# kkromberg/SpeechRecognition

Measured on AMD Instinct MI355X. Metric: frames/sec scored+decoded, higher is better.
Workload: dtype f64

## Files before the change

### speechrecognition_amd/csrc/gmm_prefilter.hip

```cpp
#include <hip/hip_runtime.h>
#include <stdint.h>

#include <algorithm>
#include <cmath>
#include <vector>

#include "kernels.h"

#ifndef SR_P16_NB
#define SR_P16_NB 4
#endif

namespace srgpu {

typedef float v4f __attribute__((ext_vector_type(4)));
static constexpr int kPWaves = 4;
static constexpr int kGroupBlocks = 8;

typedef _Float16 f16x8 __attribute__((ext_vector_type(8)));

__device__ inline uint32_t pack_f16x2(_Float16 l, _Float16 h) {
  return (uint32_t)__builtin_bit_cast(uint16_t, l) | ((uint32_t)__builtin_bit_cast(uint16_t, h) << 16);
}

template <int KS32, int NB>
__global__ __launch_bounds__(kPWaves * 64, (NB <= 2 ? 3 : 2)) void gmm_prefilter16_kernel(GmmPrefilterArgs a) {
  constexpr int kBlockBytes = KS32 * 1024;
  constexpr int kStageBytes = kGroupBlocks * kBlockBytes;
  constexpr int kChunksPerStage = kStageBytes / 1024;
  constexpr int kDmaPerWave = kChunksPerStage / kPWaves;
  static_assert(kChunksPerStage % kPWaves == 0, "every wave issues the same number of LDS-DMA pieces per stage");
  constexpr int kTileFrames = kPWaves * NB * 16;
  constexpr size_t kTileBytes = (size_t)kTileFrames * (16 * KS32) * sizeof(float);
  constexpr size_t kLdsBytes = 2 * kStageBytes > kTileBytes ? 2 * kStageBytes : kTileBytes;
  __shared__ __attribute__((aligned(1024))) unsigned char lds[kLdsBytes];

  const int lane = threadIdx.x & 63, wave = threadIdx.x >> 6;
  const int g = lane >> 4, c = lane & 15;
  uint32_t x, y;
  {
    const uint32_t id = blockIdx.x;
    if ((a.ny & 7u) == 0) { const uint32_t j = id >> 3; y = (id & 7u) + 8u * (j / a.nx); x = j % a.nx; }
    else { y = id / a.nx; x = id % a.nx; }
  }
  const uint32_t g0 = a.split_begin[y], g1 = a.split_begin[y + 1];
  const uint64_t frame0 = (uint64_t)x * kTileFrames + (uint64_t)wave * (NB * 16);

  uint4 bf[NB][KS32];
  float bnorm[NB], dbnorm[NB];
  {
    float* fl = reinterpret_cast<float*>(lds);
    const uint64_t tile_first = (uint64_t)x * kTileFrames;
    const uint64_t tile_frames = (a.n_frames - tile_first < (uint64_t)kTileFrames) ? a.n_frames - tile_first : kTileFrames;
    const uint32_t n_floats = (uint32_t)tile_frames * a.dim;
    const float* src = a.feats + tile_first * a.dim;
    for (uint32_t i = threadIdx.x; i < n_floats; i += kPWaves * 64) fl[i] = src[i];
    __syncthreads();
#pragma unroll
    for (int nb = 0; nb < NB; nb++) {
      const uint32_t row = (uint32_t)wave * (NB * 16) + nb * 16 + c;
      const bool valid = row < tile_frames;
      const float* xr = fl + (valid ? row : 0u) * a.dim;
      float n2 = 0.0f, e2 = 0.0f;
#pragma unroll
      for (int ks = 0; ks < KS32; ks++) {
        _Float16 v[8];
#pragma unroll
        for (int j = 0; j < 8; j++) {
          const uint32_t k = 32u * ks + 8u * g + j, d = k >> 1;
          const float xf = (valid && d < a.dim) ? xr[d < a.dim ? d : 0u] : 0.0f;
          const float b = (k & 1u) ? xf : xf * xf;
          n2 += b * b;
          _Float16 h = (_Float16)b;
          const float bh = (float)h;
          const float e = (k & 1u) ? xf - bh : __builtin_fmaf(xf, xf, -bh);
          e2 += e * e;
          if (valid && k >= 2u * a.dim && k < 2u * a.dim + 3u) h = (_Float16)1.0f;
          v[j] = h;
        }
        bf[nb][ks] = make_uint4(pack_f16x2(v[0], v[1]), pack_f16x2(v[2], v[3]), pack_f16x2(v[4], v[5]), pack_f16x2(v[6], v[7]));
      }
      n2 += __shfl_xor(n2, 16);
      n2 += __shfl_xor(n2, 32);
      e2 += __shfl_xor(e2, 16);
      e2 += __shfl_xor(e2, 32);
      bnorm[nb] = sqrtf(n2) * 1.0001f;
      dbnorm[nb] = fminf(sqrtf(e2) * 1.0001f, kPfRes16 * bnorm[nb]);
    }
    __syncthreads();
  }

  const unsigned char* dma_src = a.apack + (uint64_t)g0 * kStageBytes + (uint64_t)wave * 1024 + lane * 16;
  auto issue_stage = [&](int buf) {
#pragma unroll
    for (int i = 0; i < kDmaPerWave; i++) {
      const int chunk = i * kPWaves + wave;
      unsigned char* dst = lds + buf * kStageBytes + chunk * 1024;
      __builtin_amdgcn_global_load_lds((const __attribute__((address_space(1))) void*)(dma_src + i * (kPWaves * 1024)),
                                       (__attribute__((address_space(3))) void*)dst, 16, 0, 0);
    }
    dma_src += kStageBytes;
  };
  auto frag = [&](int buf, int j, int ks) -> f16x8 {
    return __builtin_bit_cast(f16x8, *reinterpret_cast<const uint4*>(lds + buf * kStageBytes + j * kBlockBytes + ks * 1024 + lane * 16));
  };

  const uint32_t n_stages = g1 - g0;
  if (n_stages > 0) issue_stage(0);
  if (n_stages > 1) issue_stage(1);
  if (n_stages > 1) __builtin_amdgcn_s_waitcnt(0x0F70 | kDmaPerWave);
  else __builtin_amdgcn_s_waitcnt(0x0F70);
  __syncthreads();
  f16x8 a_c, a_n;
  if (n_stages > 0) a_c = frag(0, 0, 0);
  uint32_t* m_ptr = a.mask + (uint64_t)g0 * a.n_frames * 4u;
  uint32_t m_off[NB];
  bool m_ok[NB];
#pragma unroll
  for (int nb = 0; nb < NB; nb++) {
    const uint64_t f = frame0 + (uint64_t)nb * 16 + c;
    m_ok[nb] = f < a.n_frames;
    m_off[nb] = (uint32_t)f * 4u + (uint32_t)g;
  }
  for (uint32_t s = 0; s < n_stages; s++) {
    const uint32_t grp = g0 + s;
    const int buf = s & 1;
    v4f ap[NB][kGroupBlocks];
#pragma unroll
    for (int j = 0; j < kGroupBlocks; j++) {
      v4f acc[NB];
#pragma unroll
      for (int nb = 0; nb < NB; nb++) acc[nb] = (v4f){0.f, 0.f, 0.f, 0.f};
#pragma unroll
      for (int ks = 0; ks < KS32; ks++) {
        if (j == kGroupBlocks - 1 && ks == KS32 - 1) {
          if (s + 1 < n_stages) {
            __builtin_amdgcn_s_waitcnt(0x0070);
            __syncthreads();
            if (s + 2 < n_stages) issue_stage(buf);
            a_n = frag(buf ^ 1, 0, 0);
          }
        } else {
          a_n = frag(buf, (ks == KS32 - 1) ? j + 1 : j, (ks == KS32 - 1) ? 0 : ks + 1);
        }
        __builtin_amdgcn_sched_barrier(0);
#pragma unroll
        for (int nb = 0; nb < NB; nb++)
          acc[nb] = __builtin_amdgcn_mfma_f32_16x16x32_f16(a_c, __builtin_bit_cast(f16x8, bf[nb][ks]), acc[nb], 0, 0, 0);
        __builtin_amdgcn_sched_barrier(0);
        a_c = a_n;
      }
#pragma unroll
      for (int nb = 0; nb < NB; nb++) ap[nb][j] = acc[nb];
    }
    const float4 lim = reinterpret_cast<const float4*>(a.grp_lim)[4u * grp + g];
#pragma unroll
    for (int nb = 0; nb < NB; nb++) {
      float amin = __builtin_huge_valf();
#pragma unroll
      for (int j = 0; j < kGroupBlocks; j += 2)
        asm("v_min3_f32 %0, %0, %1, %2\n\tv_min3_f32 %0, %0, %3, %4\n\tv_min3_f32 %0, %0, %5, %6\n\tv_min3_f32 %0, %0, %7, %8"
            : "+v"(amin)
            : "v"(ap[nb][j][0]), "v"(ap[nb][j][1]), "v"(ap[nb][j][2]), "v"(ap[nb][j][3]), "v"(ap[nb][j + 1][0]),
              "v"(ap[nb][j + 1][1]), "v"(ap[nb][j + 1][2]), "v"(ap[nb][j + 1][3]));
      if (a.chunks >= 2) { const float o = __shfl_xor(amin, 16); asm("v_min_f32 %0, %0, %1" : "+v"(amin) : "v"(o)); }
      if (a.chunks >= 4) { const float o = __shfl_xor(amin, 32); asm("v_min_f32 %0, %0, %1" : "+v"(amin) : "v"(o)); }
      const float limit = amin + __builtin_fmaf(lim.y, dbnorm[nb], __builtin_fmaf(lim.x, bnorm[nb], lim.z));
      uint32_t mask = 0;
#pragma unroll
      for (int j = kGroupBlocks - 1; j >= 1; j -= 2)
        asm("v_cmp_ngt_f32 vcc, %2, %1\n\tv_addc_co_u32 %0, vcc, %0, %0, vcc\n\t"
            "v_cmp_ngt_f32 vcc, %3, %1\n\tv_addc_co_u32 %0, vcc, %0, %0, vcc\n\t"
            "v_cmp_ngt_f32 vcc, %4, %1\n\tv_addc_co_u32 %0, vcc, %0, %0, vcc\n\t"
            "v_cmp_ngt_f32 vcc, %5, %1\n\tv_addc_co_u32 %0, vcc, %0, %0, vcc\n\t"
            "v_cmp_ngt_f32 vcc, %6, %1\n\tv_addc_co_u32 %0, vcc, %0, %0, vcc\n\t"
            "v_cmp_ngt_f32 vcc, %7, %1\n\tv_addc_co_u32 %0, vcc, %0, %0, vcc\n\t"
            "v_cmp_ngt_f32 vcc, %8, %1\n\tv_addc_co_u32 %0, vcc, %0, %0, vcc\n\t"
            "v_cmp_ngt_f32 vcc, %9, %1\n\tv_addc_co_u32 %0, vcc, %0, %0, vcc"
            : "+v"(mask)
            : "v"(limit), "v"(ap[nb][j][3]), "v"(ap[nb][j][2]), "v"(ap[nb][j][1]), "v"(ap[nb][j][0]), "v"(ap[nb][j - 1][3]),
              "v"(ap[nb][j - 1][2]), "v"(ap[nb][j - 1][1]), "v"(ap[nb][j - 1][0])
            : "vcc");
      if (m_ok[nb]) m_ptr[m_off[nb]] = mask;
    }
    m_ptr += a.n_frames * 4u;
  }
}

__global__ void fp16_denormal_probe_kernel(float* out) {
  const int lane = threadIdx.x;
  f16x8 a = {0, 0, 0, 0, 0, 0, 0, 0}, b = {0, 0, 0, 0, 0, 0, 0, 0};
  if (lane < 16) { a[0] = (_Float16)9.5367431640625e-7f; b[0] = (_Float16)1024.0f; }
  v4f acc = {0.f, 0.f, 0.f, 0.f};
  acc = __builtin_amdgcn_mfma_f32_16x16x32_f16(a, b, acc, 0, 0, 0);
  out[lane] = acc[0];
}

hipError_t probe_fp16_denormals(hipStream_t stream, bool* preserved) {
  float* d = nullptr;
  hipError_t e = hipMalloc(reinterpret_cast<void**>(&d), 64 * sizeof(float));
  if (e != hipSuccess) return e;
  hipLaunchKernelGGL(fp16_denormal_probe_kernel, dim3(1), dim3(64), 0, stream, d);
  float h[64];
  e = hipGetLastError();
  if (e == hipSuccess) e = hipStreamSynchronize(stream);
  if (e == hipSuccess) e = hipMemcpy(h, d, sizeof(h), hipMemcpyDeviceToHost);
  (void)hipFree(d);
  if (e != hipSuccess) return e;
  *preserved = true;
  for (int i = 0; i < 64; i++) *preserved = *preserved && h[i] == 9.765625e-4f;
  return hipSuccess;
}

template <int KS>
__global__ void fp16_accumulation_probe_kernel(const _Float16* A, const _Float16* B, float* out) {
  constexpr int K = 32 * KS;
  const int lane = threadIdx.x, r = lane & 15, q = lane >> 4;
  v4f acc = {0.f, 0.f, 0.f, 0.f};
#pragma unroll
// ... 616 lines not shown
#pragma unroll 1
    for (uint32_t pos = 0; pos < n_left; pos += 64u) {
      const RingEntry en = nxt;
      const uint32_t n = n_left - pos < 64u ? n_left - pos : 64u;
      const uint32_t p2 = pos + 64u;
      if (p2 < n_left) nxt = sj[p2 + ((uint32_t)lane < n_left - p2 ? lane : 0)];
      batch(true, j, en, (uint32_t)lane < n);
      level2(false);
    }
  }
  level2(true);
  if (a.n_refined) {
    if (lane == 0) atomicAdd(a.n_refined, (unsigned long long)n_eval);
  }
}

__device__ inline uint32_t padded_source_dim(uint32_t k, uint32_t dim, uint32_t dp) {
  const uint32_t pairs = dim - (dim & 1u);
  return k < pairs ? k : (k == dp - 1u && (dim & 1u)) ? dim - 1u : dim;
}
__global__ void transpose_feats_kernel(const float* feats, uint64_t n_frames, uint32_t dim, uint32_t dp, uint64_t ldT, float* out, float* featsP) {
  __shared__ float tile[64][65];
  const uint64_t f0 = (uint64_t)blockIdx.x * 64;
  for (uint32_t d0 = 0; d0 < dp; d0 += 64) {
    for (uint32_t i = threadIdx.x; i < 64 * 64; i += blockDim.x) {
      const uint32_t fr = i / 64, d = i % 64;
      const uint32_t src = d0 + d < dp ? padded_source_dim(d0 + d, dim, dp) : dim;
      tile[fr][d] = (f0 + fr < n_frames && src < dim) ? feats[(f0 + fr) * dim + src] : 0.0f;
    }
    __syncthreads();
    for (uint32_t i = threadIdx.x; i < 64 * 64; i += blockDim.x) {
      const uint32_t d = i / 64, fr = i % 64;
      if (f0 + fr < n_frames && d0 + d < dp) out[(uint64_t)(d0 + d) * ldT + f0 + fr] = tile[fr][d];
    }
    if (featsP) {
      for (uint32_t i = threadIdx.x; i < 64 * 64; i += blockDim.x) {
        const uint32_t fr = i / 64, d = i % 64;
        if (f0 + fr < n_frames && d0 + d < dp) featsP[(f0 + fr) * dp + d0 + d] = tile[fr][d];
      }
    }
    __syncthreads();
  }
}

hipError_t launch_transpose_feats(const float* feats, uint64_t n_frames, uint32_t dim, uint32_t dp, uint64_t ldT, float* out, float* featsP,
                                  hipStream_t stream) {
  if (n_frames == 0) return hipSuccess;
  if (dp < dim || (dp != dim && !featsP)) return hipErrorInvalidValue;
  hipLaunchKernelGGL(transpose_feats_kernel, dim3((unsigned)((n_frames + 63) / 64)), dim3(256), 0, stream, feats, n_frames, dim, dp, ldT, out,
                     dp != dim ? featsP : nullptr);
  return hipGetLastError();
}

int gmm_refine_slots(uint32_t max_dens, uint32_t padded_dim) { return padded_dim > 39 ? 32 : max_dens <= 8 ? 8 : max_dens <= 16 ? 16 : 32; }

uint32_t gmm_refine_padded_dim(uint32_t dim) {
  static const uint32_t bounds[] = {9, 17, 25, 33, 39, 47, 55, 63};
  const uint32_t need = dim | 1u;
  for (uint32_t b : bounds)
    if (need <= b) return b;
  return 0;
}

static int refine_threads(uint32_t dp) { return dp <= 47 ? kRThreads : kRThreadsWide; }
static int refine_spw(const GmmRefineArgs& a) {
  return (size_t)(2 * a.dim + 2) * a.n_slots * 8 * 8 <= 160 * 1024 ? 8 : 4;
}
static void refine_grid(const GmmRefineArgs& a, int spw, uint32_t* n_sgroups, uint64_t* splits, uint64_t* frames_per_split) {
  const uint64_t nt = (uint64_t)refine_threads(a.dim);
  *n_sgroups = (a.n_pstates + spw - 1) / spw;
  uint64_t sp = std::max<uint64_t>(1, (512 + *n_sgroups - 1) / *n_sgroups);
  sp = std::min<uint64_t>(sp, (a.n_frames + nt - 1) / nt);
  sp = std::max<uint64_t>(sp, 1);
  *frames_per_split = (a.n_frames + sp - 1) / sp;
  *splits = *frames_per_split ? (a.n_frames + *frames_per_split - 1) / *frames_per_split : 1;
}
size_t gmm_refine_ring_words(const GmmRefineArgs& a) {
  uint32_t g; uint64_t sp, fps;
  refine_grid(a, refine_spw(a), &g, &sp, &fps);
  return (size_t)g * sp * kRWaves * kRingWave;
}

static uint32_t defer_cap_for(const GmmRefineArgs& a, int spw) {
  uint32_t g; uint64_t sp, fps;
  refine_grid(a, spw, &g, &sp, &fps);
  const uint64_t per_wave = ((fps + kRThreads - 1) / kRThreads) * 64;
  return (uint32_t)std::min<uint64_t>(((per_wave / 4 + 63) & ~(uint64_t)63) + 64, 1u << 30);
}
void gmm_refine_defer_layout(const GmmRefineArgs& a, size_t budget_bytes, uint32_t cap_limit, uint32_t* cap, size_t* n_entries,
                             size_t* n_counts) {
  *cap = 0; *n_entries = 0; *n_counts = 0;
  if (a.chunks < 2 || a.dim > 39 || a.n_slots != 32 || a.n_frames == 0) return;
  uint32_t g; uint64_t sp, fps;
  refine_grid(a, 8, &g, &sp, &fps);
  uint32_t c = defer_cap_for(a, 8);
  if (cap_limit) c = std::min(c, cap_limit);
  const size_t segs = (size_t)g * sp * kRWaves * 8;
  if (segs * c * 16 > budget_bytes) return;
  *cap = c; *n_entries = segs * c; *n_counts = segs;
}

template <int DT, int NS, int SPW, int CH, int NT, int VS = 1>
static hipError_t launch_refine_one(const GmmRefineArgs& a0, hipStream_t stream) {
  GmmRefineArgs a = a0;
  const size_t state_bytes = (size_t)(2 * DT + 2) * NS * 8;
  const size_t smem = (SPW * state_bytes + 1023) & ~(size_t)1023;
// ... 69 lines not shown
```

### speechrecognition_amd/csrc/handles.h

```cpp
#pragma once
#include <hip/hip_runtime.h>

#include <atomic>
#include <condition_variable>
#include <cstdint>
#include <map>
#include <memory>
#include <mutex>
#include <string>
#include <thread>
#include <vector>

#include "../../include/srgpu.h"
#include "host_util.h"
#include "kernels.h"

namespace srhost {
int fail(int code, const char* fmt, ...) __attribute__((format(printf, 2, 3)));
}

#define HIP_TRY(expr)                                                                             \
  do {                                                                                            \
    hipError_t e_ = (expr);                                                                       \
    if (e_ != hipSuccess) return srhost::fail(SR_EHIP, "%s: %s (%s:%d)", #expr, hipGetErrorString(e_), __FILE__, __LINE__); \
// ... 13 lines not shown
  }
  hipError_t upload(const T* src, size_t count) {
    hipError_t e = ensure(count);
    if (e != hipSuccess || count == 0) return e;
    return hipMemcpy(p, src, count * sizeof(T), hipMemcpyHostToDevice);
  }
  void release() { if (p) (void)hipFree(p); p = nullptr; n = 0; }
  void swap(DevBuf& o) { T* tp = p; p = o.p; o.p = tp; size_t tn = n; n = o.n; o.n = tn; }
  DevBuf() = default;
  DevBuf(const DevBuf&) = delete;
  DevBuf& operator=(const DevBuf&) = delete;
  ~DevBuf() { release(); }
};

struct EventPair { hipEvent_t a, b; int kind; };


struct sr_feeder;


struct CorpusSpare {
  DevBuf<float> feats;
  DevBuf<uint64_t> d_frame_off;
  DevBuf<uint32_t> utt_order, out_words, out_count, out_flags;
  DevBuf<double> tb_score;
  DevBuf<uint16_t> tb_word, tb_bkp;
  size_t bytes() const {
    return feats.n * 4 + d_frame_off.n * 8 + (utt_order.n + out_words.n + out_count.n + out_flags.n) * 4 + tb_score.n * 8 + (tb_word.n + tb_bkp.n) * 2;
  }
};
size_t corpus_spare_cap_bytes();

struct sr_model {
  int device = 0;
  uint32_t dim = 0, n_states = 0, ld = 0;
  uint64_t n_dens = 0;
  bool max_approx = true;
  DevBuf<uint32_t> dens_off;
  DevBuf<double> means, inv_vars, norm, logw;
  DevBuf<uint32_t> dens_mean, dens_var;
  std::vector<uint32_t> h_dens_off, h_dens_mean, h_dens_var;
  std::vector<double> h_means, h_inv_vars, h_norm, h_logw;
  bool mfma_packed = false, pf_packed = false;
  uint32_t n_mean = 0, n_var = 0;
  int ksteps = 0;
  uint32_t n_blocks = 0, n_groups = 0;
  DevBuf<double> apack;
  DevBuf<uint32_t> blk_meta, grp_state;
  std::vector<uint32_t> group_first_block;
  std::map<uint32_t, std::unique_ptr<DevBuf<uint32_t>>> split_tabs, pf_split_tabs;
  const uint32_t *split_cur = nullptr, *pf_split_cur = nullptr;
  uint32_t split_ny = 0;
  int pf_ks32 = 0;
  uint32_t pf_groups = 0, pf_ny = 0, max_dens = 0, pf_slots = 0, pf_chunks = 1, pf_pstates = 0;
  DevBuf<unsigned char> pf_apack;
  DevBuf<float> pf_lim, featsT, featsP;
  DevBuf<uint4> pf_defer;
  DevBuf<uint32_t> pf_defer_cnt;
  int neg_possible = -1;
  uint32_t pf_dp = 0;
  DevBuf<uint32_t> pf_mask, pf_ndens, pf_ring;
  DevBuf<double> pf_rows;
  DevBuf<unsigned long long> pf_counter;
  hipStream_t s_copy = nullptr;
  float* staging[2] = {nullptr, nullptr};
  hipEvent_t staging_free[2] = {nullptr, nullptr};
  std::atomic<bool> staging_busy{false};
  std::mutex spare_mu;
  std::unique_ptr<CorpusSpare> spare;
  std::vector<sr_corpus*> corpora;
  hipStream_t s_gmm = nullptr, s_search = nullptr;
  DevBuf<double> scores[2];
  hipEvent_t ev_scored[2] = {nullptr, nullptr}, ev_consumed[2] = {nullptr, nullptr};
  size_t chunk_frames = 0;
  bool overlap = true;
  size_t defer_budget = (size_t)32 << 30;
  uint32_t defer_cap_limit = 0;
  size_t fb_budget = (size_t)1 << 30;
  bool profiling = false;
  std::vector<EventPair> events;
  sr_profile prof{};
};

struct sr_corpus {
  sr_model* model = nullptr;
  sr_feeder* feeder = nullptr;
  uint32_t n_utts = 0;
  uint64_t n_frames = 0;
  std::vector<uint64_t> frame_off;
  DevBuf<float> feats;
  DevBuf<uint64_t> d_frame_off;
  DevBuf<uint32_t> utt_order;
  size_t order_chunk_frames = 0;
  DevBuf<double> tb_score;
  DevBuf<uint16_t> tb_word, tb_bkp;
  DevBuf<uint32_t> out_words, out_count, out_flags;
  DevBuf<unsigned char> big_ws;
  DevBuf<uint16_t> automata, out_states;
  DevBuf<uint64_t> aut_off, bp_off, al_blk_frame0;
  DevBuf<uint32_t> al_list_off, al_states, al_blk_frames, al_blk_list;
  DevBuf<uint8_t> backptr;
  DevBuf<double> out_cost, path_scores;
  DevBuf<uint64_t> pair_off;
  DevBuf<uint32_t> pair_frame, key_mean, key_var, iota, keys_sorted, pairs_sorted, row_begin;
  DevBuf<double> pair_w, acc_mean, acc_var, w_mean, w_var;
  bool acc_valid = false;
  uint32_t acc_n_mean = 0, acc_n_var = 0;
  DevBuf<unsigned char> sort_temp;
  DevBuf<double> fb_trellis, fb_item_w, fb_weight;
// ... 144 lines not shown
```

### speechrecognition_amd/csrc/kernels.h

```cpp
#pragma once
#include <hip/hip_runtime.h>
#include <stdint.h>

#include <vector>

namespace srgpu {

struct GmmMfmaArgs {
  const float* feats;
  uint64_t n_frames;
  uint32_t dim;
  const double* apack;
  const uint32_t* blk_meta;
  const uint32_t* grp_state;
  const uint32_t* split_begin;
  double* out;
  uint32_t ld;
  uint32_t nx, ny;
};
int gmm_mfma_ksteps_for_dim(uint32_t dim);
int gmm_mfma_frames_per_tile(int ksteps);
hipError_t launch_gmm_mfma(const GmmMfmaArgs& a, int ksteps, bool sum, hipStream_t stream);

struct GmmExactArgs {
  const float* feats;
  uint64_t n_frames;
  uint32_t dim;
  uint32_t n_states;
  const uint32_t* dens_off;
  const double* means;
  const double* inv_vars;
  const double* norm;
  const double* logw;
  double* out;
  uint32_t ld;
  uint32_t states_per_split;
};
hipError_t launch_gmm_exact(const GmmExactArgs& a, bool sum, uint32_t n_splits, hipStream_t stream);
struct GmmExactList {
  const uint64_t* blk_frame0;
  const uint32_t* blk_frames;
  const uint32_t* blk_list;
  const uint32_t* list_off;
  const uint32_t* states;
  uint32_t blk_first;
  uint64_t frame_base;
};
hipError_t launch_gmm_exact_listed(const GmmExactArgs& a, bool sum, const GmmExactList& L, uint32_t n_blocks, hipStream_t stream);
int gmm_exact_frames_per_block();

struct GmmPrefilterArgs {
  const float* feats;
  uint64_t n_frames;
  uint32_t dim;
  const unsigned char* apack;
  const float* grp_lim;
  const uint32_t* split_begin;
  uint32_t* mask;
  uint32_t nx, ny;
  uint32_t chunks;
};
struct PfBound { float kappa, acc, abs, sub; };
constexpr float kPfRes16 = 4.8835e-4f;
inline constexpr PfBound pf_bound(int ks32) {
  return ks32 == 4 ? PfBound{1.05e-3f, 1.6e-5f, 7.0e-7f, 3.38e-7f} : PfBound{1.05e-3f, 1.1e-5f, 6.0e-7f, 2.92e-7f};
}
struct GmmRefineArgs {
  const float* feats;
  const float* featsT;
  uint64_t n_frames, n_frames_ld;
  uint32_t dim, n_pstates, chunks;
  const uint32_t* n_dens_ps;
  const double* rows;
  uint32_t n_slots;
  const uint32_t* mask;
  double* out; uint32_t ld;
  uint64_t frames_per_split;
  unsigned long long* n_refined;
  uint32_t* ring;
  void* defer;
  uint32_t* defer_cnt;
  uint32_t defer_cap;
};
void gmm_refine_defer_layout(const GmmRefineArgs& a, size_t budget_bytes, uint32_t cap_limit, uint32_t* cap, size_t* n_entries,
                             size_t* n_counts);
size_t gmm_refine_ring_words(const GmmRefineArgs& a);
hipError_t launch_gmm_prefilter(const GmmPrefilterArgs& a, int ks32, hipStream_t stream);
int gmm_prefilter_frames_per_tile();
hipError_t probe_fp16_denormals(hipStream_t stream, bool* preserved);
hipError_t probe_fp16_accumulation(hipStream_t stream, int ks32, bool* ok, double* worst_ratio);
uint32_t gmm_refine_padded_dim(uint32_t dim);
int gmm_refine_slots(uint32_t max_dens, uint32_t padded_dim);
hipError_t launch_gmm_refine(const GmmRefineArgs& a, hipStream_t stream);
hipError_t launch_transpose_feats(const float* feats, uint64_t n_frames, uint32_t dim, uint32_t dp, uint64_t ldT, float* out, float* featsP,
                                  hipStream_t stream);

struct DecodeNet {
  uint32_t n_slots;
  uint32_t n_words;
  const uint32_t* slot_info;
  const uint32_t* slot_word;
  const uint32_t* word_end_slot;
  uint32_t silence_word;
  double tdp_loop, tdp_forward, tdp_skip;
  uint32_t silence_state;
};
static constexpr uint32_t kSlotPos0 = 1u << 16;
static constexpr uint32_t kSlotPos1 = 1u << 17;
static constexpr uint32_t kSlotEnd = 1u << 18;
static constexpr uint32_t kSlotSilState = 1u << 19;
static constexpr uint32_t kSlotSilWord = 1u << 20;
static constexpr uint32_t kSlotFirstSil = 1u << 21;
static constexpr uint32_t kSlotSingle = 1u << 22;
struct FastNet {
  uint32_t n_slots;
  const uint32_t* state;
  const uint32_t* pred;
  const uint32_t* orig;
  const uint32_t* chunk_type;
  const uint32_t* word;
  uint32_t init_slot;
  uint32_t init_is_end;
};
struct WordNet {
  const uint32_t* info;
  const uint2* states;
  const uint32_t* order;
  uint32_t nw, nt;
  uint32_t plain_len;
  uint32_t has_general;
  uint32_t init_is_end;
};
struct DecodeArgs {
  DecodeNet net;
  FastNet fast;
  WordNet words;
  const double* scores;
  uint32_t ld;
  const uint64_t* frame_off;
  uint64_t frame_base;
// ... 525 lines not shown
```

### speechrecognition_amd/csrc/srgpu_api.cpp

```cpp
#include <hip/hip_runtime.h>

#include <algorithm>
#include <cmath>
#include <cstdarg>
#include <cstdio>
#include <cstdlib>
#include <cstring>
#include <limits>
#include <map>
#include <memory>
#include <mutex>
#include <numeric>
#include <queue>
#include <set>
#include <string>
#include <vector>

#include "../../include/srgpu.h"
#include "fb_plan.h"
#include "host_util.h"
#include "kernels.h"
#include "traceback.h"

using namespace srgpu;
// ... 212 lines not shown
          const double c = (real || t == 0) ? half_value(half_bits(rest)) : 0.0;
          arow[2 * D + t] = c;
          rest -= c;
        }
        for (int ks = 0; ks < KS; ks++)
          for (uint32_t kk = 0; kk < 32; kk++) {
            const uint32_t k = 32 * ks + kk;
            const double v = arow[k];
            const uint32_t lane = r + 16 * (kk >> 3), e = kk & 7;
            ap[(b * blk_bytes) / 2 + (size_t)ks * 512 + (size_t)lane * 8 + e] = half_bits(v);
          }
      }
    }
  }
  });
  if (Cs > 1) {
    for (uint32_t st = 0; st < S; st++)
      for (int f = 0; f < kNF; f++) {
        float mxv = 0.0f;
        for (uint32_t ch = 0; ch < Cs; ch++) {
          const float v = anorm[kNF * (size_t)(st * Cs + ch) + f];
          if (!(v <= mxv)) mxv = v;
        }
        for (uint32_t ch = 0; ch < Cs; ch++) anorm[kNF * (size_t)(st * Cs + ch) + f] = mxv;
      }
  }
  HIP_TRY(m->pf_apack.upload(reinterpret_cast<const unsigned char*>(ap.data()), ap.size() * 2));
  {
    const PfBound B = pf_bound(KS);
    for (size_t slot = 0; slot < 4 * (size_t)n_groups; slot++) {
      float* v = &anorm[kNF * slot];
      const float na = v[0], nk = v[1], nd = v[2], nh = v[3];
      const float lim0 = 2.0f * (B.acc * nk + B.abs * na), lim1_norm = 2.0f * (B.kappa * na + B.abs);
      const float lim1_res = up(2.0 * ((double)nd + (double)B.acc * nh + (double)B.abs)), limd_res = up(2.0 * (1.0 + (double)B.acc) * nh);
      const bool res = (double)limd_res * kPfRes16 + lim1_res <= lim1_norm * (1.0 - 0x1p-12) &&
                       (1.0 + (double)B.acc) * (double)B.sub * nh <= (double)B.abs * na;
      v[0] = res ? lim1_res : lim1_norm;
      v[1] = res ? limd_res : 0.0f;
      v[2] = lim0;
      v[3] = 0.0f;
    }
  }
  HIP_TRY(m->pf_lim.upload(anorm.data(), anorm.size()));
  m->pf_groups = n_groups;
  m->pf_ks32 = KS;
  m->pf_ny = 0;
  return SR_OK;
}

int set_prefilter_splits(sr_model* m, uint32_t nx) {
  const uint32_t target_wgs = 16 * 768;
  uint32_t ny = (target_wgs + nx - 1) / std::max(1u, nx);
  ny = std::max(1u, std::min(ny, std::max(1u, m->pf_groups / 8)));
  if (ny >= 8) ny &= ~7u;
  auto it = m->pf_split_tabs.find(ny);
  if (it == m->pf_split_tabs.end() || !it->second || !it->second->p) {
    std::vector<uint32_t> sb(ny + 1);
    for (uint32_t y = 0; y <= ny; y++) sb[y] = (uint32_t)((uint64_t)m->pf_groups * y / ny);
    std::unique_ptr<DevBuf<uint32_t>> fresh(new DevBuf<uint32_t>());
    HIP_TRY(fresh->upload(sb.data(), sb.size()));
    it = m->pf_split_tabs.insert_or_assign(ny, std::move(fresh)).first;
  }
  m->pf_split_cur = it->second->p;
  m->pf_ny = ny;
  return SR_OK;
}

int set_splits(sr_model* m, uint32_t nx) {
  const uint32_t target_wgs = 32 * 512;
  uint32_t ny = (target_wgs + nx - 1) / std::max(1u, nx);
  ny = std::max(1u, std::min(ny, std::min(m->n_groups, std::max(1u, m->n_blocks / 32))));
  if (ny >= 8) ny &= ~7u;
  auto it = m->split_tabs.find(ny);
  if (it == m->split_tabs.end() || !it->second || !it->second->p) {
    std::vector<uint32_t> sb(ny + 1);
    for (uint32_t y = 0; y <= ny; y++) {
      const uint64_t want = (uint64_t)m->n_blocks * y / ny;
      auto it = std::lower_bound(m->group_first_block.begin(), m->group_first_block.end(), (uint32_t)want);
      sb[y] = *it;
    }
    sb[0] = 0;
    sb[ny] = m->n_blocks;
    std::unique_ptr<DevBuf<uint32_t>> fresh(new DevBuf<uint32_t>());
    HIP_TRY(fresh->upload(sb.data(), sb.size()));
    it = m->split_tabs.insert_or_assign(ny, std::move(fresh)).first;
  }
  m->split_cur = it->second->p;
  m->split_ny = ny;
  return SR_OK;
}

int prof_begin(sr_model* m, hipStream_t s, int kind, EventPair* ep) {
  if (!m->profiling) return SR_OK;
  ep->kind = kind;
  HIP_TRY(hipEventCreate(&ep->a));
  HIP_TRY(hipEventCreate(&ep->b));
  HIP_TRY(hipEventRecord(ep->a, s));
  return SR_OK;
}
int prof_end(sr_model* m, hipStream_t s, EventPair* ep) {
  if (!m->profiling) return SR_OK;
  HIP_TRY(hipEventRecord(ep->b, s));
  m->events.push_back(*ep);
  return SR_OK;
}

int resolve_dense_kernel(const sr_model* m, int gmm_kernel) {
  if (gmm_kernel == SR_GMM_DEFAULT) gmm_kernel = m->max_approx ? SR_GMM_PREFILTER : SR_GMM_MFMA;
  if (gmm_kernel == SR_GMM_MFMA && m->ksteps == 0) gmm_kernel = SR_GMM_EXACT;
  return gmm_kernel;
}

GmmRefineArgs refine_shape(const sr_model* m, uint64_t n_frames) {
  GmmRefineArgs ra{};
  ra.n_frames = n_frames; ra.dim = m->pf_dp; ra.n_pstates = m->pf_pstates; ra.n_slots = m->pf_slots; ra.chunks = m->pf_chunks;
  return ra;
}
struct DeferLayout { uint32_t cap; size_t n_e, n_c; };
DeferLayout defer_layout(const sr_model* m, uint64_t n_frames) {
  DeferLayout d;
  gmm_refine_defer_layout(refine_shape(m, n_frames), m->defer_budget, m->defer_cap_limit, &d.cap, &d.n_e, &d.n_c);
  return d;
}

int reserve_scoring(sr_model* m, int gmm_kernel, uint64_t n_max) {
  gmm_kernel = resolve_dense_kernel(m, gmm_kernel);
  if ((gmm_kernel == SR_GMM_MFMA && !m->mfma_packed) || (gmm_kernel == SR_GMM_PREFILTER && !m->pf_packed)) {
    int rc = srhost::ensure_host_tables(m);
    if (rc) return rc;
  }
  if (gmm_kernel == SR_GMM_MFMA && !m->mfma_packed) {
    int rc = pack_model(m, m->h_dens_off.data(), m->h_means.data(), m->h_inv_vars.data(), m->h_norm.data(), m->h_logw.data());
    if (rc) return rc;
    m->mfma_packed = true;
  }
  if (gmm_kernel == SR_GMM_PREFILTER && !m->pf_packed) {
    int rc = pack_prefilter(m, m->h_dens_off.data(), m->h_means.data(), m->h_inv_vars.data(), m->h_norm.data(), m->h_logw.data());
    if (rc) return rc;
    m->pf_packed = true;
  }
  if (gmm_kernel == SR_GMM_PREFILTER && m->pf_ks32 > 0 && n_max > 0) {
    const uint64_t ldT = (n_max + 63) & ~(uint64_t)63;
    const size_t want_T = (size_t)ldT * m->pf_dp, want_mask = (size_t)((m->pf_groups + 1u) & ~1u) * n_max * 4;
    const size_t want_P = m->pf_dp != m->dim ? (size_t)n_max * m->pf_dp + 4 : 0;
    const size_t want_ring = gmm_refine_ring_words(refine_shape(m, n_max));
    if (want_T > m->featsT.n || want_P > m->featsP.n || want_mask > m->pf_mask.n || want_ring > m->pf_ring.n) HIP_TRY(hipStreamSynchronize(m->s_gmm));
    HIP_TRY(m->featsT.ensure(want_T));
    if (want_P) HIP_TRY(m->featsP.ensure(want_P));
    const DeferLayout dl = defer_layout(m, n_max);
    if (dl.n_e > m->pf_defer.n || dl.n_c > m->pf_defer_cnt.n) HIP_TRY(hipStreamSynchronize(m->s_gmm));
    if (dl.n_e) { HIP_TRY(m->pf_defer.ensure(dl.n_e)); HIP_TRY(m->pf_defer_cnt.ensure(dl.n_c)); }
    HIP_TRY(m->pf_mask.ensure(want_mask));
    HIP_TRY(m->pf_ring.ensure(want_ring));
  }
  return SR_OK;
}

int launch_scoring(sr_model* m, const float* d_feats, uint64_t n_frames, int gmm_kernel, double* d_out) {
  if (n_frames == 0) return SR_OK;
  gmm_kernel = resolve_dense_kernel(m, gmm_kernel);
  EventPair ep{};
  {
    int rc = reserve_scoring(m, gmm_kernel, n_frames);
    if (rc) return rc;
  }
  if (gmm_kernel == SR_GMM_MFMA) {
    const uint32_t tile = gmm_mfma_frames_per_tile(m->ksteps);
    const uint32_t nx = (uint32_t)((n_frames + tile - 1) / tile);
    int rc = set_splits(m, nx);
    if (rc) return rc;
    GmmMfmaArgs a{};
    a.feats = d_feats; a.n_frames = n_frames; a.dim = m->dim;
    a.apack = m->apack.p; a.blk_meta = m->blk_meta.p; a.grp_state = m->grp_state.p; a.split_begin = m->split_cur;
    a.out = d_out; a.ld = m->ld; a.nx = nx; a.ny = m->split_ny;
    if ((rc = prof_begin(m, m->s_gmm, 0, &ep))) return rc;
    HIP_TRY(launch_gmm_mfma(a, m->ksteps, !m->max_approx, m->s_gmm));
    if ((rc = prof_end(m, m->s_gmm, &ep))) return rc;
  } else if (gmm_kernel == SR_GMM_PREFILTER && m->pf_ks32 > 0) {
    const uint32_t tile = gmm_prefilter_frames_per_tile();
    const uint32_t nx = (uint32_t)((n_frames + tile - 1) / tile);
    int rc = set_prefilter_splits(m, nx);
    if (rc) return rc;
    const uint64_t ldT = (n_frames + 63) & ~(uint64_t)63;
    GmmPrefilterArgs pa{};
    pa.feats = d_feats; pa.n_frames = n_frames; pa.dim = m->dim;
    pa.apack = m->pf_apack.p; pa.grp_lim = m->pf_lim.p; pa.split_begin = m->pf_split_cur;
    pa.mask = m->pf_mask.p; pa.nx = nx; pa.ny = m->pf_ny; pa.chunks = std::min(4u, m->pf_chunks);
    GmmRefineArgs ra = refine_shape(m, n_frames);
    const bool padded = m->pf_dp != m->dim;
    ra.feats = padded ? m->featsP.p : d_feats; ra.featsT = m->featsT.p; ra.n_frames_ld = ldT;
    ra.n_dens_ps = m->pf_ndens.p; ra.rows = m->pf_rows.p;
    ra.mask = m->pf_mask.p; ra.out = d_out; ra.ld = m->ld;
    ra.n_refined = m->profiling ? m->pf_counter.p : nullptr;
    ra.ring = m->pf_ring.p;
    const DeferLayout dl = defer_layout(m, n_frames);
    if (dl.cap && dl.n_e <= m->pf_defer.n && dl.n_c <= m->pf_defer_cnt.n) { ra.defer = m->pf_defer.p; ra.defer_cnt = m->pf_defer_cnt.p; ra.defer_cap = dl.cap; }
    if (m->profiling) m->prof.refined_pairs += n_frames * (uint64_t)m->n_states;
    EventPair ep_p{}, ep_r{};
    if ((rc = prof_begin(m, m->s_gmm, 0, &ep))) return rc;
    if ((rc = prof_begin(m, m->s_gmm, 2, &ep_p))) return rc;
    HIP_TRY(launch_transpose_feats(d_feats, n_frames, m->dim, m->pf_dp, ldT, m->featsT.p, padded ? m->featsP.p : nullptr, m->s_gmm));
    HIP_TRY(launch_gmm_prefilter(pa, m->pf_ks32, m->s_gmm));
    if ((rc = prof_end(m, m->s_gmm, &ep_p))) return rc;
    if ((rc = prof_begin(m, m->s_gmm, 3, &ep_r))) return rc;
    HIP_TRY(launch_gmm_refine(ra, m->s_gmm));
    if ((rc = prof_end(m, m->s_gmm, &ep_r))) return rc;
    if ((rc = prof_end(m, m->s_gmm, &ep))) return rc;
  } else if (gmm_kernel == SR_GMM_EXACT || gmm_kernel == SR_GMM_PREFILTER) {
    GmmExactArgs a{};
    a.feats = d_feats; a.n_frames = n_frames; a.dim = m->dim; a.n_states = m->n_states;
    a.dens_off = m->dens_off.p; a.means = m->means.p; a.inv_vars = m->inv_vars.p; a.norm = m->norm.p; a.logw = m->logw.p;
    a.out = d_out; a.ld = m->ld;
    const uint32_t nx = (uint32_t)((n_frames + 255) / 256);
    uint32_t ny = std::max(1u, std::min(m->n_states, (4096 + nx - 1) / nx));
    a.states_per_split = (m->n_states + ny - 1) / ny;
    ny = (m->n_states + a.states_per_split - 1) / a.states_per_split;
    int rc;
    if ((rc = prof_begin(m, m->s_gmm, 0, &ep))) return rc;
    HIP_TRY(launch_gmm_exact(a, !m->max_approx, ny, m->s_gmm));
    if ((rc = prof_end(m, m->s_gmm, &ep))) return rc;
  } else {
    return fail(SR_EINVAL, "unknown gmm_kernel %d", gmm_kernel);
  }
  if (m->profiling) m->prof.gmm_flops += 4.0 * m->dim * (double)m->n_dens * (double)n_frames;
  return SR_OK;
}

using srplan::Chunk;
std::vector<Chunk> make_chunks(const sr_corpus* c, size_t chunk_frames) {
  std::vector<Chunk> out;
  const uint64_t total = c->n_frames;
  const uint64_t n_target = std::max<uint64_t>(1, (total + chunk_frames - 1) / std::max<size_t>(1, chunk_frames));
  const uint64_t even = (total + n_target - 1) / n_target;
  uint32_t u = 0;
  while (u < c->n_utts) {
    uint32_t v = u + 1;
    while (v < c->n_utts && c->frame_off[v + 1] - c->frame_off[u] <= chunk_frames && c->frame_off[v] - c->frame_off[u] < even) v++;
    out.push_back({u, v, c->frame_off[u], c->frame_off[v]});
    u = v;
  }
  return out;
}

int ensure_utt_order(sr_model* m, sr_corpus* c, const std::vector<Chunk>& chunks) {
  if (c->order_chunk_frames == m->chunk_frames && c->utt_order.p) return SR_OK;
  std::vector<uint32_t> order(c->n_utts);
  for (uint32_t u = 0; u < c->n_utts; u++) order[u] = u;
  for (const Chunk& ch : chunks)
    std::stable_sort(order.begin() + ch.u0, order.begin() + ch.u1, [&](uint32_t a, uint32_t b) {
      return c->frame_off[a + 1] - c->frame_off[a] > c->frame_off[b + 1] - c->frame_off[b];
    });
  HIP_TRY(c->utt_order.upload(order.data(), order.size()));
  c->order_chunk_frames = m->chunk_frames;
  return SR_OK;
// ... 183 lines not shown
}

namespace srhost {

int model_shell(int device, uint32_t dim, uint32_t n_states, const uint32_t* dens_off, int max_approx, sr_model** out) {
  *out = nullptr;
  if (!dens_off) return fail(SR_EINVAL, "null model table");
  if (dim == 0 || n_states == 0) return fail(SR_EINVAL, "dim and n_states must be positive");
  const int ks = gmm_mfma_ksteps_for_dim(dim);
  if (dim > 160) return fail(SR_ELIMIT, "dim %u unsupported (max 160: the exact kernel keeps a workgroup's frames in LDS)", dim);
  if (dens_off[0] != 0) return fail(SR_EINVAL, "dens_off[0] must be 0");
  for (uint32_t s = 0; s < n_states; s++)
    if (dens_off[s + 1] < dens_off[s]) return fail(SR_EINVAL, "dens_off must be non-decreasing (state %u)", s);
  const uint64_t C = dens_off[n_states];
  if (C >= (1ull << 31)) return fail(SR_ELIMIT, "too many densities");
  int ndev = 0;
  if (hipGetDeviceCount(&ndev) != hipSuccess || ndev == 0) return fail(SR_ENODEV, "no HIP device visible");
  if (device < 0 || device >= ndev) return fail(SR_EINVAL, "device %d out of range (0..%d)", device, ndev - 1);
  hipDeviceProp_t prop;
  HIP_TRY(hipGetDeviceProperties(&prop, device));
  if (strncmp(prop.gcnArchName, "gfx950", 6) != 0)
    return fail(SR_ENODEV, "device %d is %s; libsrgpu is built for gfx950 (MI355X) only", device, prop.gcnArchName);
  HIP_TRY(hipSetDevice(device));
  sr_model* m = new sr_model();
  std::unique_ptr<sr_model, int (*)(sr_model*)> own(m, sr_model_destroy);
  m->device = device; m->dim = dim; m->n_states = n_states; m->n_dens = C; m->max_approx = max_approx != 0;
  m->ksteps = ks;
  m->ld = (n_states + 7u) & ~7u;
  hipError_t e;
  if ((e = hipStreamCreateWithFlags(&m->s_gmm, hipStreamNonBlocking)) != hipSuccess ||
      (e = hipStreamCreateWithFlags(&m->s_search, hipStreamNonBlocking)) != hipSuccess)
    return fail(SR_EHIP, "hipStreamCreate: %s", hipGetErrorString(e));
  for (int i = 0; i < 2; i++)
    if ((e = hipEventCreateWithFlags(&m->ev_scored[i], hipEventDisableTiming)) != hipSuccess ||
        (e = hipEventCreateWithFlags(&m->ev_consumed[i], hipEventDisableTiming)) != hipSuccess)
      return fail(SR_EHIP, "hipEventCreate: %s", hipGetErrorString(e));
  if ((e = m->dens_off.upload(dens_off, n_states + 1)) != hipSuccess) return fail(SR_EHIP, "model upload: %s", hipGetErrorString(e));
  uint32_t mx = 0;
  for (uint32_t s = 0; s < n_states; s++) mx = std::max(mx, dens_off[s + 1] - dens_off[s]);
  m->max_dens = std::max(1u, mx);
  m->h_dens_off.assign(dens_off, dens_off + n_states + 1);
  const char* env = getenv("SRGPU_SCORE_CHUNK_MB");
  size_t chunk_bytes = (size_t)49152 << 20;
  {
    size_t free_b = 0, total_b = 0;
    if (hipMemGetInfo(&free_b, &total_b) == hipSuccess && total_b) chunk_bytes = std::min(chunk_bytes, total_b / 6);
  }
  if (env) chunk_bytes = (size_t)atol(env) << 20;
  m->chunk_frames = std::max<size_t>(1, chunk_bytes / ((size_t)m->ld * sizeof(double)));
  m->chunk_frames = std::min<size_t>(m->chunk_frames, ((size_t)1 << 32) / (4 * (size_t)dim) - 128);
  if (const char* ov = getenv("SRGPU_OVERLAP")) m->overlap = atoi(ov) != 0;
  if (const char* e = getenv("SRGPU_DEFER_MB")) m->defer_budget = (size_t)strtoull(e, nullptr, 10) << 20;
  if (const char* e = getenv("SRGPU_FB_MB")) m->fb_budget = std::max<size_t>(1, (size_t)strtoull(e, nullptr, 10)) << 20;
  if (const char* e = getenv("SRGPU_DEFER_CAP")) m->defer_cap_limit = std::max(1u, (uint32_t)strtoul(e, nullptr, 10));
  *out = own.release();
  return SR_OK;
}

int ensure_host_tables(sr_model* m) {
  const size_t C = m->n_dens, D = m->dim;
  if (m->h_norm.size() == C && m->h_means.size() == C * D) return SR_OK;
  m->h_means.resize(C * D); m->h_inv_vars.resize(C * D); m->h_norm.resize(C); m->h_logw.resize(C);
  if (C == 0) return SR_OK;
  HIP_TRY(hipMemcpy(m->h_means.data(), m->means.p, C * D * sizeof(double), hipMemcpyDeviceToHost));
  HIP_TRY(hipMemcpy(m->h_inv_vars.data(), m->inv_vars.p, C * D * sizeof(double), hipMemcpyDeviceToHost));
  HIP_TRY(hipMemcpy(m->h_norm.data(), m->norm.p, C * sizeof(double), hipMemcpyDeviceToHost));
  HIP_TRY(hipMemcpy(m->h_logw.data(), m->logw.p, C * sizeof(double), hipMemcpyDeviceToHost));
  return SR_OK;
}

int may_go_negative(sr_model* m, bool* out) {
  if (m->neg_possible < 0) {
    const size_t C = m->n_dens;
    std::vector<double> norm_l, logw_l;
    const double *norm = m->h_norm.data(), *logw = m->h_logw.data();
    if (m->h_norm.size() != C || m->h_logw.size() != C) {
      norm_l.resize(C); logw_l.resize(C);
      if (C) {
        HIP_TRY(hipMemcpy(norm_l.data(), m->norm.p, C * sizeof(double), hipMemcpyDeviceToHost));
        HIP_TRY(hipMemcpy(logw_l.data(), m->logw.p, C * sizeof(double), hipMemcpyDeviceToHost));
      }
      norm = norm_l.data(); logw = logw_l.data();
    }
    bool neg = false;
    for (uint32_t s = 0; s < m->n_states && !neg; s++) {
      const uint32_t c0 = m->h_dens_off[s], c1 = m->h_dens_off[s + 1];
      const double slack = m->max_approx ? 0.0 : std::log((double)std::max(1u, c1 - c0)) + 1e-6;
      for (uint32_t c = c0; c < c1; c++)
        if (!(norm[c] - logw[c] - slack >= 0.0)) { neg = true; break; }
    }
    if (!neg && m->h_inv_vars.size() == C * (size_t)m->dim)
      for (double iv : m->h_inv_vars)
        if (!(iv >= 0.0)) { neg = true; break; }
    m->neg_possible = neg ? 1 : 0;
  }
  *out = m->neg_possible == 1;
  return SR_OK;
}

}

extern "C" {

int sr_model_create(int device, uint32_t dim, uint32_t n_states, const uint32_t* dens_off, const double* means,
                    const double* inv_vars, const double* norm, const double* logw, int max_approx, sr_model** out) {
  return guarded(__func__, [&]() -> int {
// ... 3338 lines not shown
```

Baseline: 13.94 million.

## Precompute prefilter fp16 B-fragments and norms once per frame in a separate kernel

Moves the per-frame fp16 fragment packing and norm computation out of the prefilter kernel into a new pre-pass kernel that writes fragments and norms to global buffers. Previously every state-split block (ny per frame tile) recomputed them from features staged through LDS. The prefilter now loads them directly, which shrinks its LDS footprint to the double-buffered stage and removes a __syncthreads pair. It also swaps shfl_xor for ds_bpermute with precomputed addresses and adds an env override for the split count. The cost is an extra kernel launch plus global writes and reads of the fragment buffer.

```diff
diff --git a/speechrecognition_amd/csrc/gmm_prefilter.hip b/speechrecognition_amd/csrc/gmm_prefilter.hip
--- a/speechrecognition_amd/csrc/gmm_prefilter.hip
+++ b/speechrecognition_amd/csrc/gmm_prefilter.hip
@@ -31,8 +31,7 @@
   constexpr int kDmaPerWave = kChunksPerStage / kPWaves;
   static_assert(kChunksPerStage % kPWaves == 0, "every wave issues the same number of LDS-DMA pieces per stage");
   constexpr int kTileFrames = kPWaves * NB * 16;
-  constexpr size_t kTileBytes = (size_t)kTileFrames * (16 * KS32) * sizeof(float);
-  constexpr size_t kLdsBytes = 2 * kStageBytes > kTileBytes ? 2 * kStageBytes : kTileBytes;
+  constexpr size_t kLdsBytes = 2 * kStageBytes;
   __shared__ __attribute__((aligned(1024))) unsigned char lds[kLdsBytes];
 
   const int lane = threadIdx.x & 63, wave = threadIdx.x >> 6;
@@ -48,47 +47,22 @@
 
   uint4 bf[NB][KS32];
   float bnorm[NB], dbnorm[NB];
-  {
-    float* fl = reinterpret_cast<float*>(lds);
-    const uint64_t tile_first = (uint64_t)x * kTileFrames;
-    const uint64_t tile_frames = (a.n_frames - tile_first < (uint64_t)kTileFrames) ? a.n_frames - tile_first : kTileFrames;
-    const uint32_t n_floats = (uint32_t)tile_frames * a.dim;
-    const float* src = a.feats + tile_first * a.dim;
-    for (uint32_t i = threadIdx.x; i < n_floats; i += kPWaves * 64) fl[i] = src[i];
-    __syncthreads();
-#pragma unroll
-    for (int nb = 0; nb < NB; nb++) {
-      const uint32_t row = (uint32_t)wave * (NB * 16) + nb * 16 + c;
-      const bool valid = row < tile_frames;
-      const float* xr = fl + (valid ? row : 0u) * a.dim;
-      float n2 = 0.0f, e2 = 0.0f;
-#pragma unroll
-      for (int ks = 0; ks < KS32; ks++) {
-        _Float16 v[8];
-#pragma unroll
-        for (int j = 0; j < 8; j++) {
-          const uint32_t k = 32u * ks + 8u * g + j, d = k >> 1;
-          const float xf = (valid && d < a.dim) ? xr[d < a.dim ? d : 0u] : 0.0f;
-          const float b = (k & 1u) ? xf : xf * xf;
-          n2 += b * b;
-          _Float16 h = (_Float16)b;
-          const float bh = (float)h;
-          const float e = (k & 1u) ? xf - bh : __builtin_fmaf(xf, xf, -bh);
-          e2 += e * e;
-          if (valid && k >= 2u * a.dim && k < 2u * a.dim + 3u) h = (_Float16)1.0f;
-          v[j] = h;
-        }
-        bf[nb][ks] = make_uint4(pack_f16x2(v[0], v[1]), pack_f16x2(v[2], v[3]), pack_f16x2(v[4], v[5]), pack_f16x2(v[6], v[7]));
-      }
-      n2 += __shfl_xor(n2, 16);
-      n2 += __shfl_xor(n2, 32);
-      e2 += __shfl_xor(e2, 16);
-      e2 += __shfl_xor(e2, 32);
-      bnorm[nb] = sqrtf(n2) * 1.0001f;
-      dbnorm[nb] = fminf(sqrtf(e2) * 1.0001f, kPfRes16 * bnorm[nb]);
-    }
-    __syncthreads();
-  }
+#pragma unroll
+  for (int nb = 0; nb < NB; nb++) {
+    const uint64_t f = frame0 + (uint64_t)nb * 16 + c;
+    const bool valid = f < a.n_frames;
+    const uint4* src = a.bfrag + (valid ? f : 0u) * (4 * KS32) + g;
+#pragma unroll
+    for (int ks = 0; ks < KS32; ks++) {
+      const uint4 v = src[4 * ks];
+      bf[nb][ks] = valid ? v : make_uint4(0u, 0u, 0u, 0u);
+    }
+    const float2 nn = a.bnorms[valid ? f : 0u];
+    bnorm[nb] = valid ? nn.x : 0.0f;
+    dbnorm[nb] = valid ? nn.y : 0.0f;
+  }
+  int xor16 = (lane ^ 16) << 2, xor32 = (lane ^ 32) << 2;
+  asm volatile("" : "+v"(xor16), "+v"(xor32));
 
   const unsigned char* dma_src = a.apack + (uint64_t)g0 * kStageBytes + (uint64_t)wave * 1024 + lane * 16;
   auto issue_stage = [&](int buf) {
@@ -163,8 +137,8 @@
             : "+v"(amin)
             : "v"(ap[nb][j][0]), "v"(ap[nb][j][1]), "v"(ap[nb][j][2]), "v"(ap[nb][j][3]), "v"(ap[nb][j + 1][0]),
               "v"(ap[nb][j + 1][1]), "v"(ap[nb][j + 1][2]), "v"(ap[nb][j + 1][3]));
-      if (a.chunks >= 2) { const float o = __shfl_xor(amin, 16); asm("v_min_f32 %0, %0, %1" : "+v"(amin) : "v"(o)); }
-      if (a.chunks >= 4) { const float o = __shfl_xor(amin, 32); asm("v_min_f32 %0, %0, %1" : "+v"(amin) : "v"(o)); }
+      if (a.chunks >= 2) { const float o = __builtin_bit_cast(float, __builtin_amdgcn_ds_bpermute(xor16, __builtin_bit_cast(int, amin))); asm("v_min_f32 %0, %0, %1" : "+v"(amin) : "v"(o)); }
+      if (a.chunks >= 4) { const float o = __builtin_bit_cast(float, __builtin_amdgcn_ds_bpermute(xor32, __builtin_bit_cast(int, amin))); asm("v_min_f32 %0, %0, %1" : "+v"(amin) : "v"(o)); }
       const float limit = amin + __builtin_fmaf(lim.y, dbnorm[nb], __builtin_fmaf(lim.x, bnorm[nb], lim.z));
       uint32_t mask = 0;
 #pragma unroll
@@ -887,6 +861,61 @@
   return hipGetLastError();
 }
 
+template <int KS32>
+__global__ __launch_bounds__(256) void prefilter_operands_kernel(const float* feats, uint64_t n_frames, uint32_t dim, uint4* bfrag, float2* bnorms) {
+  const int lane = threadIdx.x & 63, wave = threadIdx.x >> 6;
+  const int g = lane >> 4, c = lane & 15;
+  const uint64_t f = (uint64_t)blockIdx.x * 64 + (uint64_t)wave * 16 + c;
+  const bool valid = f < n_frames;
+  const float* xr = feats + (valid ? f : 0u) * dim;
+  uint4 bf[KS32];
+  float n2 = 0.0f, e2 = 0.0f;
+#pragma unroll
+  for (int ks = 0; ks < KS32; ks++) {
+    _Float16 v[8];
+#pragma unroll
+    for (int j = 0; j < 8; j++) {
+      const uint32_t k = 32u * ks + 8u * g + j, d = k >> 1;
+      const float xf = (valid && d < dim) ? xr[d < dim ? d : 0u] : 0.0f;
+      const float b = (k & 1u) ? xf : xf * xf;
+      n2 += b * b;
+      _Float16 h = (_Float16)b;
+      const float bh = (float)h;
+      const float e = (k & 1u) ? xf - bh : __builtin_fmaf(xf, xf, -bh);
+      e2 += e * e;
+      if (valid && k >= 2u * dim && k < 2u * dim + 3u) h = (_Float16)1.0f;
+      v[j] = h;
+    }
+    bf[ks] = make_uint4(pack_f16x2(v[0], v[1]), pack_f16x2(v[2], v[3]), pack_f16x2(v[4], v[5]), pack_f16x2(v[6], v[7]));
+  }
+  n2 += __shfl_xor(n2, 16);
+  n2 += __shfl_xor(n2, 32);
+  e2 += __shfl_xor(e2, 16);
+  e2 += __shfl_xor(e2, 32);
+  const float bnorm = sqrtf(n2) * 1.0001f;
+  const float dbnorm = fminf(sqrtf(e2) * 1.0001f, kPfRes16 * bnorm);
+  if (valid) {
+#pragma unroll
+    for (int ks = 0; ks < KS32; ks++) bfrag[f * (4 * KS32) + 4 * ks + g] = bf[ks];
+    if (g == 0) bnorms[f] = make_float2(bnorm, dbnorm);
+  }
+}
+
+hipError_t launch_prefilter_operands(const GmmPrefilterArgs& a, int ks32, hipStream_t stream) {
+  if (a.n_frames == 0) return hipSuccess;
+  const dim3 grid((unsigned)((a.n_frames + 63) / 64)), block(256);
+  uint4* bfrag = const_cast<uint4*>(a.bfrag);
+  float2* bnorms = const_cast<float2*>(a.bnorms);
+  switch (ks32) {
+    case 1: hipLaunchKernelGGL(prefilter_operands_kernel<1>, grid, block, 0, stream, a.feats, a.n_frames, a.dim, bfrag, bnorms); break;
+    case 2: hipLaunchKernelGGL(prefilter_operands_kernel<2>, grid, block, 0, stream, a.feats, a.n_frames, a.dim, bfrag, bnorms); break;
+    case 3: hipLaunchKernelGGL(prefilter_operands_kernel<3>, grid, block, 0, stream, a.feats, a.n_frames, a.dim, bfrag, bnorms); break;
+    case 4: hipLaunchKernelGGL(prefilter_operands_kernel<4>, grid, block, 0, stream, a.feats, a.n_frames, a.dim, bfrag, bnorms); break;
+    default: return hipErrorInvalidValue;
+  }
+  return hipGetLastError();
+}
+
 int gmm_refine_slots(uint32_t max_dens, uint32_t padded_dim) { return padded_dim > 39 ? 32 : max_dens <= 8 ? 8 : max_dens <= 16 ? 16 : 32; }
 
 uint32_t gmm_refine_padded_dim(uint32_t dim) {
diff --git a/speechrecognition_amd/csrc/handles.h b/speechrecognition_amd/csrc/handles.h
--- a/speechrecognition_amd/csrc/handles.h
+++ b/speechrecognition_amd/csrc/handles.h
@@ -89,9 +89,12 @@
   const uint32_t *split_cur = nullptr, *pf_split_cur = nullptr;
   uint32_t split_ny = 0;
   int pf_ks32 = 0;
+  uint32_t pf_ny_force = 0;
   uint32_t pf_groups = 0, pf_ny = 0, max_dens = 0, pf_slots = 0, pf_chunks = 1, pf_pstates = 0;
   DevBuf<unsigned char> pf_apack;
   DevBuf<float> pf_lim, featsT, featsP;
+  DevBuf<uint4> pf_bfrag;
+  DevBuf<float2> pf_bnorms;
   DevBuf<uint4> pf_defer;
   DevBuf<uint32_t> pf_defer_cnt;
   int neg_possible = -1;
diff --git a/speechrecognition_amd/csrc/kernels.h b/speechrecognition_amd/csrc/kernels.h
--- a/speechrecognition_amd/csrc/kernels.h
+++ b/speechrecognition_amd/csrc/kernels.h
@@ -59,6 +59,8 @@
   uint32_t* mask;
   uint32_t nx, ny;
   uint32_t chunks;
+  const uint4* bfrag;
+  const float2* bnorms;
 };
 struct PfBound { float kappa, acc, abs, sub; };
 constexpr float kPfRes16 = 4.8835e-4f;
@@ -86,6 +88,7 @@
                              size_t* n_counts);
 size_t gmm_refine_ring_words(const GmmRefineArgs& a);
 hipError_t launch_gmm_prefilter(const GmmPrefilterArgs& a, int ks32, hipStream_t stream);
+hipError_t launch_prefilter_operands(const GmmPrefilterArgs& a, int ks32, hipStream_t stream);
 int gmm_prefilter_frames_per_tile();
 hipError_t probe_fp16_denormals(hipStream_t stream, bool* preserved);
 hipError_t probe_fp16_accumulation(hipStream_t stream, int ks32, bool* ok, double* worst_ratio);
diff --git a/speechrecognition_amd/csrc/srgpu_api.cpp b/speechrecognition_amd/csrc/srgpu_api.cpp
--- a/speechrecognition_amd/csrc/srgpu_api.cpp
+++ b/speechrecognition_amd/csrc/srgpu_api.cpp
@@ -288,6 +288,7 @@
   const uint32_t target_wgs = 16 * 768;
   uint32_t ny = (target_wgs + nx - 1) / std::max(1u, nx);
   ny = std::max(1u, std::min(ny, std::max(1u, m->pf_groups / 8)));
+  if (m->pf_ny_force) ny = std::min(m->pf_ny_force, std::max(1u, m->pf_groups));
   if (ny >= 8) ny &= ~7u;
   auto it = m->pf_split_tabs.find(ny);
   if (it == m->pf_split_tabs.end() || !it->second || !it->second->p) {
@@ -380,8 +381,13 @@
     const size_t want_T = (size_t)ldT * m->pf_dp, want_mask = (size_t)((m->pf_groups + 1u) & ~1u) * n_max * 4;
     const size_t want_P = m->pf_dp != m->dim ? (size_t)n_max * m->pf_dp + 4 : 0;
     const size_t want_ring = gmm_refine_ring_words(refine_shape(m, n_max));
-    if (want_T > m->featsT.n || want_P > m->featsP.n || want_mask > m->pf_mask.n || want_ring > m->pf_ring.n) HIP_TRY(hipStreamSynchronize(m->s_gmm));
+    const size_t want_bf = (size_t)n_max * 4 * m->pf_ks32, want_bn = (size_t)n_max;
+    if (want_T > m->featsT.n || want_P > m->featsP.n || want_mask > m->pf_mask.n || want_ring > m->pf_ring.n || want_bf > m->pf_bfrag.n ||
+        want_bn > m->pf_bnorms.n)
+      HIP_TRY(hipStreamSynchronize(m->s_gmm));
     HIP_TRY(m->featsT.ensure(want_T));
+    HIP_TRY(m->pf_bfrag.ensure(want_bf));
+    HIP_TRY(m->pf_bnorms.ensure(want_bn));
     if (want_P) HIP_TRY(m->featsP.ensure(want_P));
     const DeferLayout dl = defer_layout(m, n_max);
     if (dl.n_e > m->pf_defer.n || dl.n_c > m->pf_defer_cnt.n) HIP_TRY(hipStreamSynchronize(m->s_gmm));
@@ -422,6 +428,7 @@
     pa.feats = d_feats; pa.n_frames = n_frames; pa.dim = m->dim;
     pa.apack = m->pf_apack.p; pa.grp_lim = m->pf_lim.p; pa.split_begin = m->pf_split_cur;
     pa.mask = m->pf_mask.p; pa.nx = nx; pa.ny = m->pf_ny; pa.chunks = std::min(4u, m->pf_chunks);
+    pa.bfrag = m->pf_bfrag.p; pa.bnorms = m->pf_bnorms.p;
     GmmRefineArgs ra = refine_shape(m, n_frames);
     const bool padded = m->pf_dp != m->dim;
     ra.feats = padded ? m->featsP.p : d_feats; ra.featsT = m->featsT.p; ra.n_frames_ld = ldT;
@@ -436,6 +443,7 @@
     if ((rc = prof_begin(m, m->s_gmm, 0, &ep))) return rc;
     if ((rc = prof_begin(m, m->s_gmm, 2, &ep_p))) return rc;
     HIP_TRY(launch_transpose_feats(d_feats, n_frames, m->dim, m->pf_dp, ldT, m->featsT.p, padded ? m->featsP.p : nullptr, m->s_gmm));
+    HIP_TRY(launch_prefilter_operands(pa, m->pf_ks32, m->s_gmm));
     HIP_TRY(launch_gmm_prefilter(pa, m->pf_ks32, m->s_gmm));
     if ((rc = prof_end(m, m->s_gmm, &ep_p))) return rc;
     if ((rc = prof_begin(m, m->s_gmm, 3, &ep_r))) return rc;
@@ -725,6 +733,7 @@
   if (const char* ov = getenv("SRGPU_OVERLAP")) m->overlap = atoi(ov) != 0;
   if (const char* e = getenv("SRGPU_DEFER_MB")) m->defer_budget = (size_t)strtoull(e, nullptr, 10) << 20;
   if (const char* e = getenv("SRGPU_FB_MB")) m->fb_budget = std::max<size_t>(1, (size_t)strtoull(e, nullptr, 10)) << 20;
+  if (const char* e = getenv("SRGPU_PF_SPLITS")) m->pf_ny_force = (uint32_t)strtoul(e, nullptr, 10);
   if (const char* e = getenv("SRGPU_DEFER_CAP")) m->defer_cap_limit = std::max(1u, (uint32_t)strtoul(e, nullptr, 10));
   *out = own.release();
   return SR_OK;
```

Result: no change. 13.89 million (median of 3 runs) (-0.3%).
